# itailang/geometric_adv

Hardware: AMD Instinct MI355X
Metric: attack-iterations/sec (B=32, N=2048) at 1/2/4/8 GPUs; Chamfer rel-err vs ref (higher is better)
Workload: dtype f32 (encoder products: f16x2); 1 GPU; BASELINE configs[1]: B=32 random clouds x N=2048, output-space attack (chamfer/chamfer, dist_weight 1.0, lr 0.01), one batch per GPU; batch_per_gpu=32, n_points=2048, global_batch=32, parallelism=batches sharded, dp1, no data-path collective, ranks=1, collective_backend=none, collective_world=1

## Files before the change

### geometric_adv_amd/adv_ae.py

```python
import ctypes as C
import time

import numpy as np
import torch

from . import _lib
from .adversary import init_pert_value
from .autoencoder import PointNetAE


class Configuration:

    def __init__(self, batch_size, n_points, weights, loss="chamfer", loss_adv_type="chamfer",
                 loss_dist_type="chamfer", dist_weight_list=(1.0,), max_point_pert_weight=0.0,
                 max_point_dist_weight=0.0, num_iterations=500, num_iterations_thresh=400,
                 learning_rate=0.01, ae_name="autoencoder", emd_weight=0.0, verbose=False, batch_slots=1,
                 chamfer_prune=True, emd_reference_weights=False, recompute_backward=False, separate_adam=False,
                 chamfer_kernel="auto", encoder_backward="auto", emd_dense_levels=False, encoder_arith=None, loss_in_scan=True):
        self.batch_size = int(batch_size)
        self.n_input = [int(n_points), 3]
        self.n_output = [int(n_points), 3]
        self.weights = weights
        self.loss = loss
        self.loss_adv_type = loss_adv_type
# ... 153 lines not shown
        f = lambda *s: torch.empty(s, dtype=torch.float32, device=dev)
        i = lambda *s: torch.empty(s, dtype=torch.int32, device=dev)
        out = dict(pert=f(B, n, 3), adv=f(B, n, 3), recon=f(B, n, 3), latent=f(B, 128), grad=f(B, n, 3),
                   idx_r1=i(B, n), idx_r2=i(B, n), idx_a1=i(B, n), idx_a2=i(B, n))
        with torch.cuda.device(dev):
            _lib.check(_lib.lib().geoadv_attack_peek(self._h, *[_lib.ptr(out[k]) for k in
                       ("pert", "adv", "recon", "latent", "grad", "idx_r1", "idx_r2", "idx_a1", "idx_a2")],
                       _lib.stream_handle()), "attack_peek")
        if self.ae.bneck != 128:
            out["latent"] = out["latent"][:, :self.ae.bneck].contiguous()
        return out

    def _test_loss_form(self, form):
        _lib.check(_lib.lib().geoadv_attack_test_loss_form(self._h, int(form)), "attack_test_loss_form")

    def _test_loss_state(self):
        B, n, dev = self.B, self.n, self.device
        f = lambda *s: torch.empty(s, dtype=torch.float32, device=dev)
        out = dict(g_recon=f(B, n, 3), g_dist=f(B, n, 3), losses=f(8, B), dist_r1=f(B, n), dist_a1=f(B, n))
        with torch.cuda.device(dev):
            _lib.check(_lib.lib().geoadv_attack_test_loss_state(self._h, *[_lib.ptr(out[k]) for k in
                       ("g_recon", "g_dist", "losses", "dist_r1", "dist_a1")], _lib.stream_handle()), "attack_test_loss_state")
        return out

    def _test_plan(self):
        plan = (C.c_int * 9)()
        jstar = torch.empty((2, self.B), dtype=torch.int32, device=self.device)
        with torch.cuda.device(self.device):
            _lib.check(_lib.lib().geoadv_attack_test_plan(self._h, plan, _lib.ptr(jstar), _lib.stream_handle()), "attack_test_plan")
        return dict(symmetric=bool(plan[0]), screened=bool(plan[1]), rtiles=plan[2], rslices=plan[3],
# ... 127 lines not shown
```

### geometric_adv_amd/csrc/ae.h

```cpp
#pragma once
#include <atomic>
#include "common.h"

namespace geoadv {

constexpr int ENC_L = GEOADV_ENC_LAYERS;

struct PackedLayer {
    const float *w;
    int K, N;
};

struct DeviceAE {
    int n_points, bneck;
    int enc_dims[ENC_L + 1];
    int dec_dims[GEOADV_DEC_LAYERS + 1];
    const float *w0;
    PackedLayer enc_fwd[ENC_L];
    PackedLayer enc_bwd[ENC_L];
    PackedLayer enc_bwd16[ENC_L];
    const unsigned *enc_x3;
    const float *enc_x3_consts;
    const unsigned *enc_h2;
    const float *enc_h2_consts;
// ... 4 lines not shown
    const float *scale[ENC_L];
    const float *shift[ENC_L];
    const float *v0, *c0;
    const float *v1, *c1;
    const float *v0t, *v1t;
    PackedLayer dec2_fwd;
    PackedLayer dec2_bwd;
    const float *c2;
};

struct FusedAdam {
    float *pert, *m, *v, *g_enc;
    const float *g_dist;
    float *grad_out;
    float alpha, one_minus_b1, one_minus_b2, eps;
};

}

namespace geoadv { int ae_range_check(const geoadv_ae *ae, hipStream_t stream, const char *who); }

struct geoadv_ae {
    geoadv::DeviceAE d;
    mutable std::atomic<int> attack_refs{0};
    void *arena;
    size_t arena_bytes;
};
```

### geometric_adv_amd/csrc/ae.hip

```cpp
#include "host_util.h"
#include <cmath>
#include "encoder_x3.h"
#include <math.h>
#include <string.h>
#include <vector>
#include <atomic>

namespace geoadv {

int launch_encoder_fwd(const DeviceAE &A, int b, const float *x, const float *pert, float *adv_out, float *pmax,
                       int *parg, int *pcnt, unsigned *masks, hipStream_t stream, hipEvent_t start = nullptr, hipEvent_t stop = nullptr,
                       const FusedAdam *fused = nullptr);
int launch_latent_decode(const DeviceAE &A, int b, const float *pmax, const int *parg, const int *pcnt, float *z,
                         int *crit, int *zcnt, int *dense, float *d1, float *d2, hipStream_t stream);
int launch_decoder_fc2(const DeviceAE &A, int b, const float *d2, float *recon, hipStream_t stream, unsigned long long *fill = nullptr,
                       size_t fill_count = 0);
int launch_latent_fc(const DeviceAE &A, int b, const float *z, float *d2, hipStream_t stream);
int encoder_tiles_max(int n);

static inline uint16_t bf16_rne(float f) {
    uint32_t u;
    memcpy(&u, &f, 4);
    if ((u & 0x7fffffffu) > 0x7f800000u) return (uint16_t)((u >> 16) | 0x40u);
    u += 0x7fffu + ((u >> 16) & 1u);
    return (uint16_t)(u >> 16);
}
static inline float bf16_value(uint16_t h) {
    const uint32_t u = (uint32_t)h << 16;
    float f;
    memcpy(&f, &u, 4);
    return f;
// ... 368 lines not shown
```

### geometric_adv_amd/csrc/attack.hip

```cpp
#include "ae.h"
#include "chamfer_sym.h"
#include "chamfer_grad.h"
#include "chamfer_grid.h"
#include "encoder_jac.h"
#include "decoder_tail.h"
#define LC_STAMP(K, I) GA_STAMP(K, I)
#include "loss_cgrad.h"
#include "host_util.h"
#include <assert.h>
#include <dlfcn.h>
#include <limits.h>
#include <math.h>
#include <stdlib.h>
#include <vector>

#pragma clang fp contract(off)

namespace geoadv {

struct ChamferScan { const float *query; const float *target; float *dist; int *idx; int nq, nt; const int *need; };
int launch_chamfer_scans(const ChamferScan *scans, int nscan, int b, hipStream_t stream);
int launch_encoder_jac(const DeviceAE &A, int b, const JacArgs &a, hipStream_t stream);
int launch_encoder_bwd_dense(const DeviceAE &A, int b, const float *adv, const float *z, const int *zcnt, const float *dz,
                             const int *dense_flag, float *g_enc, hipStream_t stream);
// ... 6 lines not shown
int launch_latent_decode_and_grid(const DeviceAE &A, int b, const float *pmax, const int *parg, const int *pcnt, float *z, int *crit,
                                  int *zcnt, int *dense, float *d1, float *d2, const float *P, const float *Q, float *gd1, int *gi1,
                                  float *gd2, int *gi2, int n, int *need, int call, const float *box, hipStream_t stream);
int launch_chamfer_grid_box(const float *Q, int b, int n, float *box, hipStream_t stream);
struct ForwardScratch {
    float *pmax; int *parg; int *pcnt; float *z; int *crit; int *zcnt; int *dense; float *d1, *d2; size_t bytes;
};
ForwardScratch carve_forward_scratch(void *base, int b, int n_points);
int launch_encoder_fwd(const DeviceAE &A, int b, const float *x, const float *pert, float *adv_out, float *pmax,
                       int *parg, int *pcnt, unsigned *masks, hipStream_t stream, hipEvent_t start = nullptr, hipEvent_t stop = nullptr,
                       const FusedAdam *fused = nullptr);
int encoder_mask_words();
int launch_latent_decode(const DeviceAE &A, int b, const float *pmax, const int *parg, const int *pcnt, float *z,
                         int *crit, int *zcnt, int *dense, float *d1, float *d2, hipStream_t stream);
int launch_decoder_fc2(const DeviceAE &A, int b, const float *d2, float *recon, hipStream_t stream, unsigned long long *fill = nullptr,
                       size_t fill_count = 0);
int launch_decoder_bwd(const DeviceAE &A, int b, const float *g_recon, const float *d1, const float *d2, float *partial,
                       float *dz, hipStream_t stream, const int *crit = nullptr, const float *jac = nullptr, const int *dense = nullptr,
                       float *g_enc = nullptr);
int decoder_bwd_chunks(const DeviceAE &A);
int launch_encoder_bwd(const DeviceAE &A, int b, const float *adv, const int *crit_rows, const float *z,
                       const int *zcnt, const float *dz, const int *dense_flag, float *g_enc, const unsigned *masks,
                       hipStream_t stream);

__global__ __launch_bounds__(256) void loss_metrics_kernel(LossArgs a) { loss_metrics_body(a, blockIdx.x, gridDim.x); }

__global__ __launch_bounds__(256) void chamfer_per_pc_kernel(int n, int m, const float *d1, const float *d2, float *out) {
    __shared__ float shf[4][8];
    __shared__ int shi[4][2];
    const int b = blockIdx.x, t = threadIdx.x;
    CloudRed r;
// ... 103 lines not shown
    out[b * 5 + 4] = best_err[b];
}

__global__ void xcd_probe_kernel(unsigned *out) {
    if (threadIdx.x == 0) {
        unsigned v;
        asm volatile("s_getreg_b32 %0, hwreg(HW_REG_XCC_ID)" : "=s"(v));
        out[blockIdx.x] = v & 0xf;
    }
}

}

using namespace geoadv;

struct geoadv_attack {
    const geoadv_ae *ae;
    geoadv_attack_config cfg;
    int B, n;
    void *arena; size_t arena_bytes;
    float *x, *gt, *tz, *w;
    float *pert, *m, *v;
    float *adv, *recon, *g_recon, *g_dist, *g_enc, *grad_last;
    float *r1, *r2, *a1, *a2; int *ir1, *ir2, *ia1, *ia2;
    ForwardScratch fs;
    float *dz, *dec_partial;
    float *losses; int *jstar;
    float *best_err, *best_metrics, *best_adv, *best_recon;
    float *emd_temp, *emd_cost, *emd_g1;
    float *sym_ws;
    unsigned long long *row64;
    int test_loss_form = 0;
    int plan[GEOADV_PLAN_COUNT] = {};
    bool cgrad_done;
    bool counted = false;
    bool chamfer_prune;
    int *need_adv[2];
    int *need_last;
    float *x_box;
    int grid_calls;
    unsigned *masks;
    float *jac;
    bool jac_valid;
    unsigned *tail_ready;
    unsigned tail_epoch;
    unsigned *loss_done;
    unsigned loss_target;
// ... 96 lines not shown
    f.loss_fused = (adv_chamfer || dist_chamfer) && !max_term && n <= CG_FX_MAX_N_PLANE;
    f.merge_in_loss = f.loss_fused && adv_chamfer && dist_chamfer;
    f.jac_rides = at->jac && at->chamfer_sym;
    SymPlan plan{};
    if (at->chamfer_sym) {
        SymRequest rq{2, B, n, n, true, f.pruned, f.rides_scan, f.jac_rides};
        rq.loss = at->host_loss && f.merge_in_loss && !at->emd_temp; rq.loss_rows = 1 + 2 * H; rq.loss_force = at->host_loss_force;
        rq.defer = f.merge_in_loss; rq.packed = f.merge_in_loss && at->row64 != nullptr;
        rq.pack_from = (at->test_loss_form & 1) ? SYM_PACK_FROM + 1 : SYM_PACK_FROM;
        rq.screen = chamfer_sym_screen_on();
        plan = chamfer_sym_plan(rq);
    }
    const SymRows rows = chamfer_sym_rows(plan, at->sym_ws, at->row64);
    const bool packed = plan.rows == GEOADV_PLAN_ROWS_PACKED, hosted = plan.loss.count > 0;
    const int call = at->grid_calls;
    int *need_new = at->need_adv[f.rides_scan ? (call + 1) & 1 : 0];
    const int *need_scan = at->need_adv[f.rides_scan ? call & 1 : 0];
    if (f.pruned) { at->grid_calls++; at->need_last = need_new; }
    {
        ProfScope ps(at, GEOADV_PROF_ENCODER_FWD, st, true);
        if (int rc = launch_encoder_fwd(A, B, at->x, at->pert, (at->adv_valid && !at->adam_pending) ? nullptr : at->adv, at->fs.pmax,
                                        at->fs.parg, at->fs.pcnt, at->masks, st, ps.start(), ps.stop(),
                                        at->adam_pending ? &at->pending : nullptr)) return rc;
        at->adam_pending = false;
        at->adv_valid = true;
    }
    {
        ProfScope ps(at, GEOADV_PROF_DECODER_FWD, st);
        if (f.pruned && !f.rides_scan && !f.rides_latent) {
            if (int rc = launch_chamfer_grid(at->adv, at->x, at->a1, at->ia1, at->a2, at->ia2, B, n, need_new, call, at->x_box, st)) return rc;
        }
        if (f.rides_latent) {
            if (int rc = launch_latent_decode_and_grid(A, B, at->fs.pmax, at->fs.parg, at->fs.pcnt, at->fs.z, at->fs.crit, at->fs.zcnt,
                                                       at->fs.dense, at->fs.d1, at->fs.d2, at->adv, at->x, at->a1, at->ia1, at->a2,
                                                       at->ia2, n, need_new, call, at->x_box, st)) return rc;
        } else if (int rc = launch_latent_decode(A, B, at->fs.pmax, at->fs.parg, at->fs.pcnt, at->fs.z, at->fs.crit, at->fs.zcnt,
                                                 at->fs.dense, at->fs.d1, at->fs.d2, st)) return rc;
        if (int rc = launch_decoder_fc2(A, B, at->fs.d2, at->recon, st, packed ? at->row64 : nullptr, packed ? 2 * (size_t)B * n : 0)) return rc;
    }
    const JacArgs jargs{n, at->masks, at->fs.crit, at->fs.z, at->fs.dense, at->jac};
    at->jac_valid = f.jac_rides;
    if (at->jac && !f.jac_rides && at->cfg.encoder_backward == GEOADV_ENC_BWD_JACOBIAN) {
        ProfScope ps(at, GEOADV_PROF_ENCODER_BWD, st);
        if (int rc = launch_encoder_jac(A, B, jargs, st)) return rc;
        at->jac_valid = true;
    }
    LossArgs la;
    CGradArgs ca;
    int np = 0;
    la.n = n; la.loss_adv_type = at->cfg.loss_adv_type; la.loss_dist_type = at->cfg.loss_dist_type;
    la.mp_pert_w = at->cfg.max_point_pert_weight; la.mp_dist_w = at->cfg.max_point_dist_weight;
    la.r1 = at->r1; la.r2 = at->r2; la.a1 = at->a1; la.a2 = at->a2; la.pert = at->pert;
    la.z = at->fs.z; la.tz = at->tz; la.w = at->w; la.losses = at->losses; la.jstar = at->jstar;
// ... 78 lines not shown
int launch_cgrad(const CGradProblem *pr, int np, int B, int n, hipStream_t st) {
    CGradArgs ca;
    for (int i = 0; i < np; ++i) ca.pr[i] = pr[i];
    ca.n = n; ca.P = pow2_ge(n);
    if (!cgrad_step_sorted(n)) {
        const int H = cgrad_fx_parts(n);
        chamfer_grad_attack_fx_kernel<<<dim3(B, np * H), CGA_THREADS, cgrad_fx_lds_bytes(n), st>>>(ca, H);
        GA_LAUNCH_CHECK();
        return GEOADV_OK;
    }
    chamfer_grad_attack_kernel<<<dim3(B, np), CGA_THREADS, sizeof(unsigned) * (size_t)ca.P * (ca.P <= CG_TERMS_MAX_P ? 4 : 1), st>>>(ca);
    GA_LAUNCH_CHECK();
    return GEOADV_OK;
}

int do_step(geoadv_attack *at, hipStream_t st) {
    const DeviceAE &A = at->ae->d;
    const int B = at->B, n = at->n;
    const bool adv_chamfer = at->cfg.loss_adv_type == GEOADV_LOSS_ADV_CHAMFER;
    const bool dist_chamfer = at->cfg.loss_dist_type == GEOADV_LOSS_DIST_CHAMFER;
    const CGradProblem p_recon{at->recon, at->gt, at->ir1, at->ir2, at->g_recon, nullptr, nullptr, 0.f};
    const CGradProblem p_dist{at->adv, at->x, at->ia1, at->ia2, at->g_dist, at->w, at->jstar, at->cfg.max_point_dist_weight};
    if (!at->cgrad_done) {
        ProfScope ps(at, GEOADV_PROF_LOSS_GRAD, st);
        CGradProblem pr[2];
        int np = 0;
        if (adv_chamfer) pr[np++] = p_recon;
        if (dist_chamfer) pr[np++] = p_dist;
        if (np)
            if (int rc = launch_cgrad(pr, np, B, n, st)) return rc;
    }
// ... 20 lines not shown
            ta.adv = at->adv; ta.z = at->fs.z; ta.zcnt = at->fs.zcnt; ta.dense_flag = at->fs.dense; ta.g_enc = at->g_enc;
            ta.ready = at->tail_ready; ta.epoch = ++at->tail_epoch; ta.spin_timeout = reinterpret_cast<int *>(at->tail_ready + B);
            if (int rc = launch_decoder_tail_dense(A, ta, st)) return rc;
            }
        } else if (int rc = launch_decoder_bwd(A, B, at->g_recon, at->fs.d1, at->fs.d2, at->dec_partial, at->dz, st)) return rc;
    }
    if (!(adv_chamfer && at->jac_valid)) {
        ProfScope ps(at, GEOADV_PROF_ENCODER_BWD, st);
        if (int rc = launch_encoder_bwd(A, B, at->adv, at->fs.crit, at->fs.z, at->fs.zcnt, at->dz, at->fs.dense, at->g_enc, at->masks, st))
            return rc;
    }
    {
        const float beta1 = 0.9f, beta2 = 0.999f;
        const float alpha = at->cfg.learning_rate * sqrtf(1.0f - at->beta2_pow) / (1.0f - at->beta1_pow);
        if (at->fuse_adam && dist_chamfer) {
            at->pending = FusedAdam{at->pert, at->m, at->v, at->g_enc, at->g_dist, at->grad_last, alpha, 1.0f - beta1, 1.0f - beta2, 1e-8f};
            at->adam_pending = true;
        } else {
            ProfScope ps(at, GEOADV_PROF_ADAM, st);
            AdamArgs aa;
            aa.n = n; aa.B = B; aa.pert = at->pert; aa.m = at->m; aa.v = at->v; aa.g_enc = at->g_enc;
            aa.g_dist = dist_chamfer ? at->g_dist : nullptr; aa.w = at->w; aa.losses = at->losses; aa.jstar = at->jstar;
            aa.loss_dist_type = at->cfg.loss_dist_type; aa.mp_pert_w = at->cfg.max_point_pert_weight;
            aa.alpha = alpha;
            aa.one_minus_b1 = 1.0f - beta1; aa.one_minus_b2 = 1.0f - beta2; aa.eps = 1e-8f;
            aa.grad_out = at->grad_last; aa.x = at->x; aa.adv_out = at->adv;
            const size_t total = (size_t)B * n * 3;
            adam_kernel<<<(unsigned)((total + 255) / 256), 256, 0, st>>>(aa);
            GA_LAUNCH_CHECK();
        }
        at->beta1_pow *= beta1;
// ... 183 lines not shown
    GA_HIP(hipMemsetAsync(at->best_adv, 0, 4 * bn3, st));
    GA_HIP(hipMemsetAsync(at->best_recon, 0, 4 * bn3, st));
    at->fwd_valid = false; at->adv_valid = false;
    return GEOADV_OK;
}

extern "C" int geoadv_attack_run(geoadv_attack *at, int first_iteration, int iterations, int thresh,
                                 float *metrics_hist, void *stream) {
    GA_REQUIRE(at && first_iteration >= 0 && iterations >= 0, "attack_run: bad arguments");
    hipStream_t st = as_stream(stream);
    at->prof_stream = st;
    if (iterations == 0) return GEOADV_OK;
    if (!at->fwd_valid)
        if (int rc = do_forward(at, nullptr, 0, st)) return rc;
    for (int i = 0; i < iterations; ++i) {
        if (int rc = do_step(at, st)) return rc;
        const int it = first_iteration + i;
        const int keep = (it + 1) >= thresh ? 1 : 0;
        float *slot = metrics_hist ? metrics_hist + (size_t)i * 6 * at->B : nullptr;
        if (int rc = do_forward(at, slot, keep, st)) return rc;
    }
    return GEOADV_OK;
}

extern "C" int geoadv_attack_get_best(geoadv_attack *at, const float *target_ae_loss_ref, float *metrics, float *adv,
                                      float *recon, void *stream) {
    GA_REQUIRE(at, "attack_get_best: null handle");
    hipStream_t st = as_stream(stream);
    const size_t bn3 = (size_t)at->B * at->n * 3;
    if (metrics) {
        GA_REQUIRE(target_ae_loss_ref, "attack_get_best: target_ae_loss_ref is required for the metrics");
// ... 3 lines not shown
    }
    if (adv) GA_HIP(hipMemcpyAsync(adv, at->best_adv, 4 * bn3, hipMemcpyDeviceToDevice, st));
    if (recon) GA_HIP(hipMemcpyAsync(recon, at->best_recon, 4 * bn3, hipMemcpyDeviceToDevice, st));
    return GEOADV_OK;
}

extern "C" int geoadv_attack_set_source_search(geoadv_attack *at, int on) {
    GA_REQUIRE(at, "attack_set_source_search: null handle");
    at->chamfer_prune = on != 0;
    return GEOADV_OK;
}

extern "C" int geoadv_attack_test_loss_form(geoadv_attack *at, int form) {
    GA_REQUIRE(at && form >= 0 && form <= 3, "attack_test_loss_form: bad arguments");
    at->test_loss_form = form;
    return GEOADV_OK;
}

extern "C" int geoadv_attack_test_loss_state(geoadv_attack *at, float *g_recon, float *g_dist, float *losses, float *dist_r1,
                                             float *dist_a1, void *stream) {
    GA_REQUIRE(at, "attack_test_loss_state: null handle");
    hipStream_t st = as_stream(stream);
    const size_t bn3 = 4 * (size_t)at->B * at->n * 3, bn = 4 * (size_t)at->B * at->n;
    if (at->adam_pending || !at->fwd_valid)
        if (int rc = do_forward(at, nullptr, 0, st)) return rc;
    GA_REQUIRE(at->cgrad_done || !(g_recon || g_dist), "attack_test_loss_state: this configuration forms the Chamfer gradients in the step");
    if (g_recon) GA_HIP(hipMemcpyAsync(g_recon, at->g_recon, bn3, hipMemcpyDeviceToDevice, st));
    if (g_dist) GA_HIP(hipMemcpyAsync(g_dist, at->g_dist, bn3, hipMemcpyDeviceToDevice, st));
    if (losses) GA_HIP(hipMemcpyAsync(losses, at->losses, 4 * 8 * (size_t)at->B, hipMemcpyDeviceToDevice, st));
    if (dist_r1) GA_HIP(hipMemcpyAsync(dist_r1, at->r1, bn, hipMemcpyDeviceToDevice, st));
// ... 100 lines not shown
```

### geometric_adv_amd/csrc/decoder.hip

```cpp
#include "ae.h"
#include "decoder_tail.h"
#include "chamfer_grid.h"
#include <limits.h>

namespace geoadv {

int encoder_tiles(const DeviceAE &A, int b);

typedef float f32x16 __attribute__((ext_vector_type(16)));
typedef float f32x4 __attribute__((ext_vector_type(4)));
__device__ __forceinline__ int acc_row16(int reg, int h) { return (reg & 3) + 8 * (reg >> 2) + 4 * h; }

template <int THREADS, int PARTS = 1>
__device__ __forceinline__ void latent_decode_block(const DeviceAE &A, int tiles, const float *pmax, const int *parg,
                                                    const int *pcnt, float *z, int *crit, int *zcnt,
                                                    int *dense, float *d1, float *d2, const int b, const int part_id = 0) {
    __shared__ float gm[8][128];
    __shared__ int ga[8][128], gk[8][128];
    __shared__ float zs[128];
    __shared__ float hs[256];
    __shared__ float part[4][256];
    __shared__ int tie;
    const int t = threadIdx.x;
    GA_STAMP(0, 0);
// ... 109 lines not shown
__global__ __launch_bounds__(THREADS) void latent_decode_and_grid_kernel(DeviceAE A, int tiles, const float *pmax, const int *parg,
                                                                         const int *pcnt, float *z, int *crit, int *zcnt, int *dense,
                                                                         float *d1, float *d2, int batch, GridArgs G) {
    if ((int)blockIdx.x < batch) {
        latent_decode_block<THREADS>(A, tiles, pmax, parg, pcnt, z, crit, zcnt, dense, d1, d2, blockIdx.x);
        return;
    }
    if (THREADS > GR_THREADS && threadIdx.x >= GR_THREADS) return;
    const int g = blockIdx.x - batch;
    GA_STAMP(1, 0);
    grid_nn_block<GR_MAX_N>(G, g / (2 * GR_QSPLIT), (g / GR_QSPLIT) % 2, g % GR_QSPLIT);
    GA_STAMP(1, 7);
}

__device__ __forceinline__ void decoder_fc2_block(const DeviceAE &A, int batch, const float *d2, float *out, const int cb, const int rb,
                                                  unsigned long long *fill = nullptr, size_t fill_count = 0) {
    __shared__ float part[4][16][64];
    GA_STAMP(2, 0);
    const int wave = threadIdx.x >> 6, lane = threadIdx.x & 63;
    const int h = lane >> 5, i = lane & 31;
    const PackedLayer &L = A.dec2_fwd;
    const int kg = L.K >> 3;
    const int per = kg / 4;
    int arow = rb * 32 + i;
    arow = arow < batch ? arow : batch - 1;
    const float *ap = d2 + (size_t)arow * 256 + 4 * h;
    const float4 *bp = reinterpret_cast<const float4 *>(L.w) + (size_t)cb * kg * 64 + lane;
    f32x16 acc = {};
    float4 av[8], wv[8];
#pragma unroll
    for (int u = 0; u < 8; ++u) {
// ... 1 lines not shown
        av[u] = *reinterpret_cast<const float4 *>(ap + 8 * t);
        wv[u] = bp[(size_t)t * 64];
    }
    const int ncols = A.dec_dims[GEOADV_DEC_LAYERS];
    const int col = cb * 32 + i;
    const float bias_ld = A.c2[col < ncols ? col : ncols - 1];
#pragma unroll
    for (int u = 0; u < 8; ++u) {
        if (u < per) {
            acc = __builtin_amdgcn_mfma_f32_32x32x2f32(av[u].x, wv[u].x, acc, 0, 0, 0);
            acc = __builtin_amdgcn_mfma_f32_32x32x2f32(av[u].y, wv[u].y, acc, 0, 0, 0);
            acc = __builtin_amdgcn_mfma_f32_32x32x2f32(av[u].z, wv[u].z, acc, 0, 0, 0);
            acc = __builtin_amdgcn_mfma_f32_32x32x2f32(av[u].w, wv[u].w, acc, 0, 0, 0);
        }
    }
    if (fill) {
        const size_t stride = (size_t)gridDim.x * gridDim.y * 256;
        for (size_t e = ((size_t)blockIdx.y * gridDim.x + blockIdx.x) * 256 + threadIdx.x; e < fill_count; e += stride) fill[e] = ~0ull;
    }
#pragma unroll
    for (int r = 0; r < 16; ++r) part[wave][r][lane] = acc[r];
    __syncthreads();
    {
        float p[4][4];
#pragma unroll
        for (int j = 0; j < 4; ++j)
#pragma unroll
            for (int q = 0; q < 4; ++q) p[j][q] = part[q][4 * wave + j][lane];
        const float bias = col < ncols ? bias_ld : 0.f;
        const int row0 = rb * 32 + 8 * wave + 4 * h;
        float *op = out + (size_t)row0 * ncols + col;
#pragma unroll
        for (int j = 0; j < 4; ++j) {
            const float v = ((p[j][0] + p[j][1]) + p[j][2]) + p[j][3] + bias;
            if (row0 + j < batch && col < ncols) op[(size_t)j * ncols] = v;
        }
    }
    GA_STAMP(2, 7);
}

__global__ __launch_bounds__(256) void decoder_fc2_kernel(DeviceAE A, int batch, const float *d2, float *out, unsigned long long *fill,
                                                         size_t fill_count) {
    decoder_fc2_block(A, batch, d2, out, blockIdx.x, blockIdx.y, fill, fill_count);
}

constexpr int DB_KC = 64;

__global__ __launch_bounds__(512) void decoder_fc2_bwd_kernel(DeviceAE A, int batch, const float *g_out, float *partial) {
    __shared__ __attribute__((aligned(16))) float as[32 * (DB_KC + 4)];
    GA_STAMP(3, 0);
    const int ch = blockIdx.x, rb = blockIdx.y;
    const int ncols = A.dec_dims[GEOADV_DEC_LAYERS];
    const PackedLayer &L = A.dec2_bwd;
    const int kg_total = L.K >> 3;
    const int k0 = ch * DB_KC;
    const int wave = threadIdx.x >> 6, lane = threadIdx.x & 63;
    const int h = lane >> 5, i = lane & 31;
    const int cb = wave;
// ... 86 lines not shown
            A, encoder_tiles(A, b), pmax, parg, pcnt, z, crit, zcnt, dense, d1, d2, b, G);
    else
        latent_decode_and_grid_kernel<GR_THREADS><<<blocks, GR_THREADS, chamfer_grid_lds_bytes(n), stream>>>(
            A, encoder_tiles(A, b), pmax, parg, pcnt, z, crit, zcnt, dense, d1, d2, b, G);
    GA_LAUNCH_CHECK();
    return GEOADV_OK;
}

int launch_latent_fc(const DeviceAE &A, int b, const float *z, float *d2, hipStream_t stream) {
    if (b <= 0) return GEOADV_OK;
    latent_fc_kernel<<<b, LD_THREADS, 0, stream>>>(A, z, d2);
    GA_LAUNCH_CHECK();
    return GEOADV_OK;
}

int launch_decoder_fc2(const DeviceAE &A, int b, const float *d2, float *recon, hipStream_t stream, unsigned long long *fill, size_t fill_count) {
    if (b <= 0) return GEOADV_OK;
    decoder_fc2_kernel<<<dim3(A.dec2_fwd.N / 32, cdiv(b, 32)), 256, 0, stream>>>(A, b, d2, recon, fill, fill_count);
    GA_LAUNCH_CHECK();
    return GEOADV_OK;
}

int decoder_bwd_chunks(const DeviceAE &A) { return cdiv(A.dec2_bwd.K, DB_KC); }

int launch_decoder_fc2_bwd(const DeviceAE &A, int b, const float *g_recon, float *partial, hipStream_t stream) {
    if (b <= 0) return GEOADV_OK;
    decoder_fc2_bwd_kernel<<<dim3(decoder_bwd_chunks(A), cdiv(b, 32)), 512, 0, stream>>>(A, b, g_recon, partial);
    GA_LAUNCH_CHECK();
    return GEOADV_OK;
}

int launch_decoder_bwd(const DeviceAE &A, int b, const float *g_recon, const float *d1, const float *d2, float *partial,
                       float *dz, hipStream_t stream, const int *crit, const float *jac, const int *dense, float *g_enc) {
// ... 12 lines not shown
```

### geometric_adv_amd/csrc/encoder_x3.hip

```cpp
#include "encoder_x3.h"
#include "encoder_jac.h"
#include <hip/hip_ext.h>
#include <limits.h>
#include <type_traits>

namespace geoadv {

constexpr int X3_THREADS = 256;
constexpr int X3_POINTS = 128;
constexpr int X3_RING = 4, X3_AHEAD = 3;
constexpr int X3_SLOT_STEPS = 1;
constexpr int X3_BIG_WG_PER_CU = 2;
constexpr int X3_SLOTS = X3_STEPS / X3_SLOT_STEPS;
__host__ __device__ constexpr int xp_slot_words(int np) { return X3_SLOT_STEPS * xp_step_words(np); }
static_assert(X3_STEPS % X3_SLOT_STEPS == 0, "whole slots");
#ifndef X3_SPLIT_HALVES
#define X3_SPLIT_HALVES 1
#endif
constexpr size_t x3_lds_bytes(int np, bool masks) {
    return (size_t)X3_RING * xp_slot_words(np) * 4 + sizeof(float) * X3_CONST_FLOATS + (sizeof(float) + 2 * sizeof(int)) * 4 * 128 +
           (masks ? sizeof(unsigned) * 2 * X3_POINTS * MASK_WORDS : 0);
}
static_assert(X3_BIG_WG_PER_CU * x3_lds_bytes(3, true) <= 160 * 1024, "the workgroups of a CU share its 160 KB of LDS");

// ... 41 lines not shown
    }
}
__device__ __forceinline__ void x3_store_point(const X3Point &o, float *adv_out, const FusedAdam &fa) {
    if (!o.valid) return;
#pragma unroll
    for (int a = 0; a < 3; ++a) {
        if (fa.m) {
            fa.g_enc[o.pg + a] = 0.f;
            if (fa.grad_out) fa.grad_out[o.pg + a] = o.g[a];
            fa.m[o.pg + a] = o.m[a]; fa.v[o.pg + a] = o.vv[a]; fa.pert[o.pg + a] = o.pnew[a];
        }
        if (adv_out) adv_out[o.pg + a] = o.v[a];
    }
}

__device__ __forceinline__ void x3_stage_constants(const float *consts, float *cst, int threads) {
    const float4 *src = reinterpret_cast<const float4 *>(consts);
    float4 *dst = reinterpret_cast<float4 *>(cst);
    for (int e = threadIdx.x; e < X3_CONST_FLOATS / 4; e += threads) dst[e] = src[e];
}

template <int NP, bool MASKS>
__device__ __forceinline__ void x3_layer0(const float *cst, const float (&pc)[3], int h, XP<NP> (&act1)[4], unsigned (&m01)[2], float &gmax) {
    const float4 *c4 = reinterpret_cast<const float4 *>(cst);
    m01[0] = m01[1] = 0u;
#pragma unroll
    for (int kb = 0; kb < 4; ++kb) {
        float v[8];
        unsigned m8 = 0;
        const int c0 = 16 * kb + 8 * h;
// ... 60 lines not shown
    int *reda = reinterpret_cast<int *>(redm + 4 * 128), *redc = reda + 4 * 128;
    unsigned *mtile = reinterpret_cast<unsigned *>(redc + 4 * 128);

    const int lane = threadIdx.x & 63, wave = __builtin_amdgcn_readfirstlane(threadIdx.x >> 6);
    const int p = lane & 31, h = lane >> 5;
    const int tile = blockIdx.x, b = blockIdx.y, tiles = gridDim.x;
    const int n0 = tile * X3_POINTS + wave * 32;
    const unsigned *img = xp_image(A, NPc{});
    float gmax = 0.f;
    GA_STAMP(0, 0);

    float pc[3];
    {
        X3Point pt;
        x3_load_point(n, b, n0 + p, x, pert, fa, pt);
        if (h == 0) x3_store_point(pt, adv_out, fa);
        pc[0] = pt.v[0]; pc[1] = pt.v[1]; pc[2] = pt.v[2];
    }
    x3_stage_constants(xp_consts(A, NPc{}), cst, X3_THREADS);
    __syncthreads();
    GA_STAMP(0, 1);

    auto fetch = [&](int t) {
#pragma unroll
        for (int u = 0; u < X3_SLOT_STEPS; ++u) {
            const int s = t * X3_SLOT_STEPS + u;
            const unsigned *src = img + (size_t)s * STEP_WORDS + wave * NP * X3_FRAG_WORDS + lane * 4;
            unsigned *dst = ring + (t % X3_RING) * SLOT_WORDS + u * STEP_WORDS + wave * NP * X3_FRAG_WORDS;
#pragma unroll
            for (int q = 0; q < NP; ++q) x3_glds16(src + q * X3_FRAG_WORDS, dst + q * X3_FRAG_WORDS);
        }
// ... 169 lines not shown
    const int p = lane & 31, h = lane >> 5;
    const int tile = blockIdx.x, b = blockIdx.y, tiles = gridDim.x;
    const int n0 = tile * 32;
    GA_STAMP(1, 0);
    const __amdgpu_buffer_rsrc_t wsrc = __builtin_amdgcn_make_buffer_rsrc(const_cast<unsigned *>(xp_image(A, NPc{})) + wave * NP * X3_FRAG_WORDS, 0, 0x7fffffff, 0x00020000);
    const unsigned lb = (unsigned)lane * 16u;
    float gmax = 0.f;
    XPN wr[X3S_AHEAD];
    auto fetch = [&](int s) {
#pragma unroll
        for (int q = 0; q < NP; ++q) wr[s % X3S_AHEAD].p[q] = __builtin_amdgcn_raw_buffer_load_b128(wsrc, lb, (s * STEP_WORDS + q * X3_FRAG_WORDS) * 4, 0);
    };
    if (wave == 0) {
        X3Point pt;
        x3_load_point(n, b, n0 + p, x, pert, fa, pt);
        if (h == 0) {
            x3_store_point(pt, adv_out, fa);
            pcs[p * 3] = pt.v[0]; pcs[p * 3 + 1] = pt.v[1]; pcs[p * 3 + 2] = pt.v[2];
        }
    }
    x3_stage_constants(xp_consts(A, NPc{}), cst, X3_THREADS);
#pragma unroll
    for (int s = 0; s < X3S_AHEAD; ++s) fetch(s);
    asm volatile("s_waitcnt lgkmcnt(0)" ::: "memory");
    __builtin_amdgcn_s_barrier();
    asm volatile("" ::: "memory");
    float pc[3] = {pcs[p * 3], pcs[p * 3 + 1], pcs[p * 3 + 2]};
    GA_STAMP(1, 1);

    XPN act1[4];
    {
        unsigned m01[2];
        x3_layer0<NP, MASKS>(cst, pc, h, act1, m01, gmax);
        if (MASKS && wave == 0) {
// ... 156 lines not shown
```

### geometric_adv_amd/csrc/mfma_tile.h

```cpp
#pragma once
#include "ae.h"

namespace geoadv {

typedef float f32x16 __attribute__((ext_vector_type(16)));

constexpr int ENC_THREADS = 512;

__device__ __forceinline__ int acc_row(int reg, int h) { return (reg & 3) + 8 * (reg >> 2) + 4 * h; }

__device__ __forceinline__ float4 ld_pinned(const float4 *p) {
    typedef float v4 __attribute__((ext_vector_type(4)));
    const v4 t = *reinterpret_cast<const v4 *>(p);
    return make_float4(t.x, t.y, t.z, t.w);
}

typedef unsigned u32x4 __attribute__((ext_vector_type(4)));
struct FragSrc {
    __amdgpu_buffer_rsrc_t rsrc;
    int off;
};
__device__ __forceinline__ FragSrc frag_src(const float *w, int first_kgroup) {
    return FragSrc{__builtin_amdgcn_make_buffer_rsrc(const_cast<float *>(w), 0, 0x7fffffff, 0x00020000), first_kgroup * 1024};
}
__device__ __forceinline__ FragSrc frag_at(const FragSrc &f, int kgroups) { return FragSrc{f.rsrc, f.off + kgroups * 1024}; }
__device__ __forceinline__ float4 ld_frag(const FragSrc &f, int kgroup, unsigned lane_bytes) {
    const u32x4 t = __builtin_amdgcn_raw_buffer_load_b128(f.rsrc, lane_bytes, f.off + kgroup * 1024, 0);
    return make_float4(__uint_as_float(t.x), __uint_as_float(t.y), __uint_as_float(t.z), __uint_as_float(t.w));
}
template <int RM>
__device__ __forceinline__ void mfma_group(const float4 (&a)[RM], const float4 &b, f32x16 (&acc)[RM]) {
#pragma unroll
    for (int rm = 0; rm < RM; ++rm) {
        acc[rm] = __builtin_amdgcn_mfma_f32_32x32x2f32(a[rm].x, b.x, acc[rm], 0, 0, 0);
        acc[rm] = __builtin_amdgcn_mfma_f32_32x32x2f32(a[rm].y, b.y, acc[rm], 0, 0, 0);
        acc[rm] = __builtin_amdgcn_mfma_f32_32x32x2f32(a[rm].z, b.z, acc[rm], 0, 0, 0);
        acc[rm] = __builtin_amdgcn_mfma_f32_32x32x2f32(a[rm].w, b.w, acc[rm], 0, 0, 0);
    }
}

template <int RM>
__device__ __forceinline__ void gemm_chain(const float *in, int s_in, int row0, const PackedLayer &L, int cb, int t0,
                                           int t1, f32x16 (&acc)[RM]) {
    const int lane = threadIdx.x & 63;
// ... 187 lines not shown
```

### include/geoadv.h

```cpp
#ifndef GEOADV_H
#define GEOADV_H

#include <stddef.h>

#ifdef __cplusplus
extern "C" {
#endif

#define GEOADV_OK      0
#define GEOADV_EINVAL  1
#define GEOADV_EHIP    2
#define GEOADV_ENOMEM  3
#define GEOADV_ERANGE  4

int         geoadv_version(void);
const char *geoadv_last_error(void);


int geoadv_nn_distance(int b, int n, const float *xyz1, int m, const float *xyz2,
                       float *dist1, int *idx1, float *dist2, int *idx2, void *stream);

size_t geoadv_nn_distance_sym_workspace_floats(int b, int n, int m);
int geoadv_nn_distance_sym_is_screened(int b, int n, int m);
int geoadv_set_chamfer_screen(int on);
// ... 395 lines not shown

int geoadv_attack_run(geoadv_attack *at, int first_iteration, int iterations, int thresh,
                      float *metrics_hist, void *stream);

int geoadv_attack_get_best(geoadv_attack *at, const float *target_ae_loss_ref,
                           float *metrics, float *adv, float *recon, void *stream);

int geoadv_attack_set_source_search(geoadv_attack *at, int on);

int geoadv_attack_status(geoadv_attack *at, void *stream);

int geoadv_attack_peek(geoadv_attack *at, float *pert, float *adv, float *recon, float *latent,
                       float *grad, int *idx_r1, int *idx_r2, int *idx_a1, int *idx_a2, void *stream);

int geoadv_attack_test_loss_form(geoadv_attack *at, int form);
int geoadv_attack_test_loss_state(geoadv_attack *at, float *g_recon, float *g_dist, float *losses, float *dist_r1, float *dist_a1,
                                  void *stream);
enum {
    GEOADV_PLAN_SYMMETRIC = 0,
    GEOADV_PLAN_SCREENED = 1,
    GEOADV_PLAN_RTILES = 2,
    GEOADV_PLAN_RSLICES = 3,
    GEOADV_PLAN_ROWS = 4,
    GEOADV_PLAN_LOSS = 5,
    GEOADV_PLAN_GRAD = 6,
    GEOADV_PLAN_H = 7,
    GEOADV_PLAN_RANGE = 8,
    GEOADV_PLAN_COUNT = 9
};
enum { GEOADV_PLAN_ROWS_FINAL = 0, GEOADV_PLAN_ROWS_PARTIALS = 1, GEOADV_PLAN_ROWS_PACKED = 2, GEOADV_PLAN_ROWS_MERGE_LAUNCH = 3 };
// ... 74 lines not shown
```

Before: 9194 attack-iterations/sec.

## Use wide write-through buffer stores for Adam state, skip per-step grad copy

Adam outputs in the encoder x3 kernel (m, v, pert, adv, zeroed g_enc) are now staged through LDS and written as 16-byte buffer stores with a write-through cache policy, instead of per-point scalar stores. The decoder fc2 row64 fill also uses wide write-through stores. The gradient output copy is skipped on every iteration except the last. Together these aim to cut store traffic and cache pollution, at the cost of extra LDS staging and wave barriers, plus test hooks to restore the old paths.

```diff
diff --git a/geometric_adv_amd/adv_ae.py b/geometric_adv_amd/adv_ae.py
--- a/geometric_adv_amd/adv_ae.py
+++ b/geometric_adv_amd/adv_ae.py
@@ -191,6 +191,17 @@
     def _test_loss_form(self, form):
         _lib.check(_lib.lib().geoadv_attack_test_loss_form(self._h, int(form)), "attack_test_loss_form")
 
+    def _test_store_form(self, bits):
+        _lib.check(_lib.lib().geoadv_attack_test_store_form(self._h, int(bits)), "attack_test_store_form")
+
+    def _test_adam_state(self):
+        B, n, dev = self.B, self.n, self.device
+        out = dict(m=torch.empty((B, n, 3), dtype=torch.float32, device=dev), v=torch.empty((B, n, 3), dtype=torch.float32, device=dev))
+        with torch.cuda.device(dev):
+            _lib.check(_lib.lib().geoadv_attack_test_adam_state(self._h, _lib.ptr(out["m"]), _lib.ptr(out["v"]), _lib.stream_handle()),
+                       "attack_test_adam_state")
+        return out
+
     def _test_loss_state(self):
         B, n, dev = self.B, self.n, self.device
         f = lambda *s: torch.empty(s, dtype=torch.float32, device=dev)
diff --git a/geometric_adv_amd/csrc/ae.h b/geometric_adv_amd/csrc/ae.h
--- a/geometric_adv_amd/csrc/ae.h
+++ b/geometric_adv_amd/csrc/ae.h
@@ -42,6 +42,7 @@
     const float *g_dist;
     float *grad_out;
     float alpha, one_minus_b1, one_minus_b2, eps;
+    int wide;
 };
 
 }
diff --git a/geometric_adv_amd/csrc/ae.hip b/geometric_adv_amd/csrc/ae.hip
--- a/geometric_adv_amd/csrc/ae.hip
+++ b/geometric_adv_amd/csrc/ae.hip
@@ -14,7 +14,7 @@
 int launch_latent_decode(const DeviceAE &A, int b, const float *pmax, const int *parg, const int *pcnt, float *z,
                          int *crit, int *zcnt, int *dense, float *d1, float *d2, hipStream_t stream);
 int launch_decoder_fc2(const DeviceAE &A, int b, const float *d2, float *recon, hipStream_t stream, unsigned long long *fill = nullptr,
-                       size_t fill_count = 0);
+                       size_t fill_count = 0, bool fill_write_through = false);
 int launch_latent_fc(const DeviceAE &A, int b, const float *z, float *d2, hipStream_t stream);
 int encoder_tiles_max(int n);
 
diff --git a/geometric_adv_amd/csrc/attack.hip b/geometric_adv_amd/csrc/attack.hip
--- a/geometric_adv_amd/csrc/attack.hip
+++ b/geometric_adv_amd/csrc/attack.hip
@@ -44,7 +44,7 @@
 int launch_latent_decode(const DeviceAE &A, int b, const float *pmax, const int *parg, const int *pcnt, float *z,
                          int *crit, int *zcnt, int *dense, float *d1, float *d2, hipStream_t stream);
 int launch_decoder_fc2(const DeviceAE &A, int b, const float *d2, float *recon, hipStream_t stream, unsigned long long *fill = nullptr,
-                       size_t fill_count = 0);
+                       size_t fill_count = 0, bool fill_write_through = false);
 int launch_decoder_bwd(const DeviceAE &A, int b, const float *g_recon, const float *d1, const float *d2, float *partial,
                        float *dz, hipStream_t stream, const int *crit = nullptr, const float *jac = nullptr, const int *dense = nullptr,
                        float *g_enc = nullptr);
@@ -178,6 +178,10 @@
 
 using namespace geoadv;
 
+#ifndef GA_STORE_ITEMS
+#define GA_STORE_ITEMS 7
+#endif
+
 struct geoadv_attack {
     const geoadv_ae *ae;
     geoadv_attack_config cfg;
@@ -195,6 +199,7 @@
     float *sym_ws;
     unsigned long long *row64;
     int test_loss_form = 0;
+    int test_store_form = 0;
     int plan[GEOADV_PLAN_COUNT] = {};
     bool cgrad_done;
     bool counted = false;
@@ -321,6 +326,11 @@
     const SymRows rows = chamfer_sym_rows(plan, at->sym_ws, at->row64);
     const bool packed = plan.rows == GEOADV_PLAN_ROWS_PACKED, hosted = plan.loss.count > 0;
     const int call = at->grid_calls;
+    const int store_form = at->test_store_form;
+    if (at->adam_pending) {
+        at->pending.wide = (store_form & GEOADV_STORE_FORM_PLAIN) || !(GA_STORE_ITEMS & 1) ? 0 : 1;
+        if (store_form & GEOADV_STORE_FORM_GRAD_EVERY_STEP) at->pending.grad_out = at->grad_last;
+    }
     int *need_new = at->need_adv[f.rides_scan ? (call + 1) & 1 : 0];
     const int *need_scan = at->need_adv[f.rides_scan ? call & 1 : 0];
     if (f.pruned) { at->grid_calls++; at->need_last = need_new; }
@@ -343,7 +353,8 @@
                                                        at->ia2, n, need_new, call, at->x_box, st)) return rc;
         } else if (int rc = launch_latent_decode(A, B, at->fs.pmax, at->fs.parg, at->fs.pcnt, at->fs.z, at->fs.crit, at->fs.zcnt,
                                                  at->fs.dense, at->fs.d1, at->fs.d2, st)) return rc;
-        if (int rc = launch_decoder_fc2(A, B, at->fs.d2, at->recon, st, packed ? at->row64 : nullptr, packed ? 2 * (size_t)B * n : 0)) return rc;
+        if (int rc = launch_decoder_fc2(A, B, at->fs.d2, at->recon, st, packed ? at->row64 : nullptr, packed ? 2 * (size_t)B * n : 0,
+                                        !(store_form & GEOADV_STORE_FORM_PLAIN) && (GA_STORE_ITEMS & 4))) return rc;
     }
     const JacArgs jargs{n, at->masks, at->fs.crit, at->fs.z, at->fs.dense, at->jac};
     at->jac_valid = f.jac_rides;
@@ -452,7 +463,7 @@
     return GEOADV_OK;
 }
 
-int do_step(geoadv_attack *at, hipStream_t st) {
+int do_step(geoadv_attack *at, bool want_grad, hipStream_t st) {
     const DeviceAE &A = at->ae->d;
     const int B = at->B, n = at->n;
     const bool adv_chamfer = at->cfg.loss_adv_type == GEOADV_LOSS_ADV_CHAMFER;
@@ -503,7 +514,8 @@
         const float beta1 = 0.9f, beta2 = 0.999f;
         const float alpha = at->cfg.learning_rate * sqrtf(1.0f - at->beta2_pow) / (1.0f - at->beta1_pow);
         if (at->fuse_adam && dist_chamfer) {
-            at->pending = FusedAdam{at->pert, at->m, at->v, at->g_enc, at->g_dist, at->grad_last, alpha, 1.0f - beta1, 1.0f - beta2, 1e-8f};
+            at->pending = FusedAdam{at->pert, at->m, at->v, at->g_enc, at->g_dist, want_grad || !(GA_STORE_ITEMS & 2) ? at->grad_last : nullptr, alpha,
+                                    1.0f - beta1, 1.0f - beta2, 1e-8f, 0};
             at->adam_pending = true;
         } else {
             ProfScope ps(at, GEOADV_PROF_ADAM, st);
@@ -717,7 +729,7 @@
     if (!at->fwd_valid)
         if (int rc = do_forward(at, nullptr, 0, st)) return rc;
     for (int i = 0; i < iterations; ++i) {
-        if (int rc = do_step(at, st)) return rc;
+        if (int rc = do_step(at, i + 1 == iterations, st)) return rc;
         const int it = first_iteration + i;
         const int keep = (it + 1) >= thresh ? 1 : 0;
         float *slot = metrics_hist ? metrics_hist + (size_t)i * 6 * at->B : nullptr;
@@ -751,6 +763,23 @@
 extern "C" int geoadv_attack_test_loss_form(geoadv_attack *at, int form) {
     GA_REQUIRE(at && form >= 0 && form <= 3, "attack_test_loss_form: bad arguments");
     at->test_loss_form = form;
+    return GEOADV_OK;
+}
+
+extern "C" int geoadv_attack_test_store_form(geoadv_attack *at, int bits) {
+    GA_REQUIRE(at && bits >= 0 && bits <= 7, "attack_test_store_form: bad arguments");
+    at->test_store_form = bits;
+    return GEOADV_OK;
+}
+
+extern "C" int geoadv_attack_test_adam_state(geoadv_attack *at, float *m, float *v, void *stream) {
+    GA_REQUIRE(at, "attack_test_adam_state: null handle");
+    hipStream_t st = as_stream(stream);
+    const size_t bn3 = 4 * (size_t)at->B * at->n * 3;
+    if (at->adam_pending)
+        if (int rc = do_forward(at, nullptr, 0, st)) return rc;
+    if (m) GA_HIP(hipMemcpyAsync(m, at->m, bn3, hipMemcpyDeviceToDevice, st));
+    if (v) GA_HIP(hipMemcpyAsync(v, at->v, bn3, hipMemcpyDeviceToDevice, st));
     return GEOADV_OK;
 }
 
diff --git a/geometric_adv_amd/csrc/decoder.hip b/geometric_adv_amd/csrc/decoder.hip
--- a/geometric_adv_amd/csrc/decoder.hip
+++ b/geometric_adv_amd/csrc/decoder.hip
@@ -1,5 +1,6 @@
 #include "ae.h"
 #include "decoder_tail.h"
+#include "mfma_tile.h"
 #include "chamfer_grid.h"
 #include <limits.h>
 
@@ -147,7 +148,7 @@
 }
 
 __device__ __forceinline__ void decoder_fc2_block(const DeviceAE &A, int batch, const float *d2, float *out, const int cb, const int rb,
-                                                  unsigned long long *fill = nullptr, size_t fill_count = 0) {
+                                                  unsigned long long *fill = nullptr, size_t fill_count = 0, int fill_wide = 0) {
     __shared__ float part[4][16][64];
     GA_STAMP(2, 0);
     const int wave = threadIdx.x >> 6, lane = threadIdx.x & 63;
@@ -179,7 +180,12 @@
             acc = __builtin_amdgcn_mfma_f32_32x32x2f32(av[u].w, wv[u].w, acc, 0, 0, 0);
         }
     }
-    if (fill) {
+    if (fill && fill_wide) {
+        const __amdgpu_buffer_rsrc_t dst = wt_dst(fill, (unsigned)(fill_count * 8));
+        const unsigned pairs = (unsigned)((fill_count + 1) / 2), stride = gridDim.x * gridDim.y * 256u;
+        const u32x4 ones = {~0u, ~0u, ~0u, ~0u};
+        for (unsigned e = (blockIdx.y * gridDim.x + blockIdx.x) * 256u + threadIdx.x; e < pairs; e += stride) wt_store16(ones, dst, e * 16u);
+    } else if (fill) {
         const size_t stride = (size_t)gridDim.x * gridDim.y * 256;
         for (size_t e = ((size_t)blockIdx.y * gridDim.x + blockIdx.x) * 256 + threadIdx.x; e < fill_count; e += stride) fill[e] = ~0ull;
     }
@@ -205,8 +211,8 @@
 }
 
 __global__ __launch_bounds__(256) void decoder_fc2_kernel(DeviceAE A, int batch, const float *d2, float *out, unsigned long long *fill,
-                                                         size_t fill_count) {
-    decoder_fc2_block(A, batch, d2, out, blockIdx.x, blockIdx.y, fill, fill_count);
+                                                         size_t fill_count, int fill_wide) {
+    decoder_fc2_block(A, batch, d2, out, blockIdx.x, blockIdx.y, fill, fill_count, fill_wide);
 }
 
 constexpr int DB_KC = 64;
@@ -323,9 +329,11 @@
     return GEOADV_OK;
 }
 
-int launch_decoder_fc2(const DeviceAE &A, int b, const float *d2, float *recon, hipStream_t stream, unsigned long long *fill, size_t fill_count) {
-    if (b <= 0) return GEOADV_OK;
-    decoder_fc2_kernel<<<dim3(A.dec2_fwd.N / 32, cdiv(b, 32)), 256, 0, stream>>>(A, b, d2, recon, fill, fill_count);
+int launch_decoder_fc2(const DeviceAE &A, int b, const float *d2, float *recon, hipStream_t stream, unsigned long long *fill, size_t fill_count,
+                       bool fill_write_through) {
+    if (b <= 0) return GEOADV_OK;
+    const bool wide = fill_write_through && fill_count % 2 == 0 && reinterpret_cast<uintptr_t>(fill) % 16 == 0 && fill_count * 8 < (1ull << 31);
+    decoder_fc2_kernel<<<dim3(A.dec2_fwd.N / 32, cdiv(b, 32)), 256, 0, stream>>>(A, b, d2, recon, fill, fill_count, wide ? 1 : 0);
     GA_LAUNCH_CHECK();
     return GEOADV_OK;
 }
diff --git a/geometric_adv_amd/csrc/encoder_x3.hip b/geometric_adv_amd/csrc/encoder_x3.hip
--- a/geometric_adv_amd/csrc/encoder_x3.hip
+++ b/geometric_adv_amd/csrc/encoder_x3.hip
@@ -79,6 +79,26 @@
     }
 }
 
+__device__ __forceinline__ bool x3_wide_ok(int n, int b, int n0) { return n0 + 32 <= n && (((size_t)b * n) & 3) == 0; }
+__device__ __forceinline__ void x3_store_wide(const X3Point &o, size_t first, float *adv_out, const FusedAdam &fa, float *stage, int lane) {
+    const int p = lane & 31;
+    int slot = 0;
+    auto put = [&](float *dst, const float (&val)[3]) {
+        float *s = stage + 96 * (slot++ & 3);
+        if (lane < 32) { s[3 * p] = val[0]; s[3 * p + 1] = val[1]; s[3 * p + 2] = val[2]; }
+        __builtin_amdgcn_wave_barrier();
+        typedef float f4 __attribute__((ext_vector_type(4)));
+        if (lane < 24) wt_store16(__builtin_bit_cast(u32x4, *reinterpret_cast<const f4 *>(s + 4 * lane)), wt_dst(dst + first, 384), (unsigned)lane * 16u);
+        __builtin_amdgcn_wave_barrier();
+    };
+    if (fa.m) {
+        if (lane < 24) wt_store16(u32x4{0u, 0u, 0u, 0u}, wt_dst(fa.g_enc + first, 384), (unsigned)lane * 16u);
+        if (fa.grad_out) put(fa.grad_out, o.g);
+        put(fa.m, o.m); put(fa.v, o.vv); put(fa.pert, o.pnew);
+    }
+    if (adv_out) put(adv_out, o.v);
+}
+
 __device__ __forceinline__ void x3_stage_constants(const float *consts, float *cst, int threads) {
     const float4 *src = reinterpret_cast<const float4 *>(consts);
     float4 *dst = reinterpret_cast<float4 *>(cst);
@@ -169,7 +189,8 @@
     {
         X3Point pt;
         x3_load_point(n, b, n0 + p, x, pert, fa, pt);
-        if (h == 0) x3_store_point(pt, adv_out, fa);
+        if (fa.m && fa.wide && x3_wide_ok(n, b, n0)) x3_store_wide(pt, ((size_t)b * n + n0) * 3, adv_out, fa, redm + wave * 384, lane);
+        else if (h == 0) x3_store_point(pt, adv_out, fa);
         pc[0] = pt.v[0]; pc[1] = pt.v[1]; pc[2] = pt.v[2];
     }
     x3_stage_constants(xp_consts(A, NPc{}), cst, X3_THREADS);
@@ -369,10 +390,9 @@
     if (wave == 0) {
         X3Point pt;
         x3_load_point(n, b, n0 + p, x, pert, fa, pt);
-        if (h == 0) {
-            x3_store_point(pt, adv_out, fa);
-            pcs[p * 3] = pt.v[0]; pcs[p * 3 + 1] = pt.v[1]; pcs[p * 3 + 2] = pt.v[2];
-        }
+        if (fa.m && fa.wide && x3_wide_ok(n, b, n0)) x3_store_wide(pt, ((size_t)b * n + n0) * 3, adv_out, fa, reinterpret_cast<float *>(xbuf), lane);
+        else if (h == 0) x3_store_point(pt, adv_out, fa);
+        if (h == 0) { pcs[p * 3] = pt.v[0]; pcs[p * 3 + 1] = pt.v[1]; pcs[p * 3 + 2] = pt.v[2]; }
     }
     x3_stage_constants(xp_consts(A, NPc{}), cst, X3_THREADS);
 #pragma unroll
diff --git a/geometric_adv_amd/csrc/mfma_tile.h b/geometric_adv_amd/csrc/mfma_tile.h
--- a/geometric_adv_amd/csrc/mfma_tile.h
+++ b/geometric_adv_amd/csrc/mfma_tile.h
@@ -28,6 +28,13 @@
     const u32x4 t = __builtin_amdgcn_raw_buffer_load_b128(f.rsrc, lane_bytes, f.off + kgroup * 1024, 0);
     return make_float4(__uint_as_float(t.x), __uint_as_float(t.y), __uint_as_float(t.z), __uint_as_float(t.w));
 }
+__device__ __forceinline__ __amdgpu_buffer_rsrc_t wt_dst(void *base, unsigned bytes) {
+    return __builtin_amdgcn_make_buffer_rsrc(base, 0, (int)bytes, 0x00020000);
+}
+__device__ __forceinline__ void wt_store16(const u32x4 &v, __amdgpu_buffer_rsrc_t dst, unsigned byte_off) {
+    __builtin_amdgcn_raw_buffer_store_b128(v, dst, (int)byte_off, 0, 16);
+}
+
 template <int RM>
 __device__ __forceinline__ void mfma_group(const float4 (&a)[RM], const float4 &b, f32x16 (&acc)[RM]) {
 #pragma unroll
diff --git a/include/geoadv.h b/include/geoadv.h
--- a/include/geoadv.h
+++ b/include/geoadv.h
@@ -433,6 +433,9 @@
                        float *grad, int *idx_r1, int *idx_r2, int *idx_a1, int *idx_a2, void *stream);
 
 int geoadv_attack_test_loss_form(geoadv_attack *at, int form);
+enum { GEOADV_STORE_FORM_PLAIN = 1, GEOADV_STORE_FORM_MASKS_AT_END = 2, GEOADV_STORE_FORM_GRAD_EVERY_STEP = 4 };
+int geoadv_attack_test_store_form(geoadv_attack *at, int bits);
+int geoadv_attack_test_adam_state(geoadv_attack *at, float *m, float *v, void *stream);
 int geoadv_attack_test_loss_state(geoadv_attack *at, float *g_recon, float *g_dist, float *losses, float *dist_r1, float *dist_a1,
                                   void *stream);
 enum {
```

Measured after the change: 9232 attack-iterations/sec, median of 6. Within noise of the previous version (+0.4%).
